# fevzibabaoglu/adaptive-edge-aware-jpeg

Measured on NVIDIA B200. Metric: encode+decode megapixels/sec, higher is better.
Workload: dtype f32

## Files before the change

adaptive-edge-aware-jpeg_b200/csrc/canny.cu:

```cuda
#include "aeaj_internal.cuh"

namespace {

__constant__ float c_bil_color[256];
__constant__ float c_bil_space[13];
__constant__ int c_bil_dy[13];
__constant__ int c_bil_dx[13];

struct ClaheGeom { int th, tw, clip; float lutScale, inv_th, inv_tw; };
__host__ __device__ inline ClaheGeom clahe_geom(int h, int w) {
    int eh = h, ew = w;
    if ((w % 4) != 0 || (h % 4) != 0) { eh = h + (4 - h % 4); ew = w + (4 - w % 4); }
    ClaheGeom g;
    g.th = eh / 4; g.tw = ew / 4;
    int area = g.th * g.tw;
    g.lutScale = 255.0f / (float)area;
    int clip = (int)(0.75 * area / 256);
    g.clip = clip < 1 ? 1 : clip;
    g.inv_th = 1.0f / (float)g.th; g.inv_tw = 1.0f / (float)g.tw;
    return g;
}

constexpr int HIST_ROWS = 32;
__device__ __forceinline__ void hist_add16(unsigned int* wh, uint4 q) {
    const unsigned w[4] = {q.x, q.y, q.z, q.w};
    int prev = w[0] & 0xff, cnt = 0;
#pragma unroll
    for (int k = 0; k < 16; k++) {
        const int v = (w[k >> 2] >> (8 * (k & 3))) & 0xff;
        if (v == prev) cnt++;
        else { atomicAdd(&wh[prev], (unsigned)cnt); prev = v; cnt = 1; }
    }
    atomicAdd(&wh[prev], (unsigned)cnt);
}
__global__ void __launch_bounds__(256) k_clahe_hist(const PlaneDesc* __restrict__ planes) {
    const PlaneDesc& P = planes[blockIdx.z];
    ClaheGeom g = clahe_geom(P.h, P.w);
    const int tile = blockIdx.y, ty = tile >> 2, tx = tile & 3;
    const int r0 = blockIdx.x * HIST_ROWS;
    if (r0 >= g.th) return;
    __shared__ unsigned int wh[8][256];
    for (int i = threadIdx.x; i < 8 * 256; i += 256) (&wh[0][0])[i] = 0;
    __syncthreads();
    const int warp = threadIdx.x >> 5, lane = threadIdx.x & 31;
    const int r1 = min(r0 + HIST_ROWS, g.th);
    const uint8_t* src = P.u8a;
    unsigned int* my = wh[warp];
    const int cx0 = tx * g.tw, cx1 = cx0 + g.tw;
    const int band_hi = (P.ry1 >= P.h) ? 4 * g.th : P.ry1;
    for (int r = r0 + warp; r < r1; r += 8) {
        const int gy = ty * g.th + r;
        if (gy < P.ry0 || gy >= band_hi) continue;
        const int sy = reflect101(gy, P.h);
        const uint8_t* rowp = src + (size_t)sy * P.w;
        const int xa = cx0, xb = min(cx1, P.w);
        if (xa < xb) {
            const int head = min((int)((16 - ((uintptr_t)(rowp + xa) & 15)) & 15), xb - xa);
            const int nvec = (xb - xa - head) >> 4;
            const int tail0 = xa + head + nvec * 16;
            for (int x = xa + lane; x < xa + head; x += 32) atomicAdd(&my[rowp[x]], 1u);
            for (int x = tail0 + lane; x < xb; x += 32) atomicAdd(&my[rowp[x]], 1u);
            const uint4* vp = reinterpret_cast<const uint4*>(rowp + xa + head);
            for (int c = lane; c < nvec; c += 32) hist_add16(my, __ldg(vp + c));
        }
        for (int x = max(cx0, P.w) + lane; x < cx1; x += 32) atomicAdd(&my[rowp[reflect101(x, P.w)]], 1u);
    }
    __syncthreads();
    unsigned s = 0;
#pragma unroll
    for (int k = 0; k < 8; k++) s += wh[k][threadIdx.x];
    if (s) atomicAdd(&P.clahe_hist[tile * 256 + threadIdx.x], s);
}

__device__ __forceinline__ unsigned peer_sum(const unsigned int* mine, const PeerSet& peers) {
    unsigned s = 0;
    for (int r = 0; r < peers.world; r++)
        s += (r == peers.rank) ? *mine : __ldcv(reinterpret_cast<const unsigned int*>(reinterpret_cast<const char*>(mine) + peers.delta[r]));
    return s;
}

__global__ void __launch_bounds__(256) k_clahe_lut(const PlaneDesc* __restrict__ planes, const __grid_constant__ PeerSet peers) {
    const PlaneDesc& P = planes[blockIdx.y];
    ClaheGeom g = clahe_geom(P.h, P.w);
    const int tile = blockIdx.x, i = threadIdx.x;
    __shared__ int red[256];
    int hv = (int)peer_sum(&P.clahe_hist[tile * 256 + i], peers);
    int excess = hv > g.clip ? hv - g.clip : 0;
    hv = hv > g.clip ? g.clip : hv;
    red[i] = excess;
    __syncthreads();
    for (int s = 128; s > 0; s >>= 1) { if (i < s) red[i] += red[i + s]; __syncthreads(); }
    int clipped = red[0];
    __syncthreads();
    int redist = clipped / 256, residual = clipped - redist * 256;
    hv += redist;
    if (residual != 0) {
        int step = 256 / residual; if (step < 1) step = 1;
        if ((i % step) == 0 && (i / step) < residual) hv++;
    }
    red[i] = hv;
    __syncthreads();
    for (int off = 1; off < 256; off <<= 1) {
        int t = (i >= off) ? red[i - off] : 0;
        __syncthreads();
        red[i] += t;
        __syncthreads();
    }
    int v = __float2int_rn(__fmul_rn((float)red[i], g.lutScale));
    P.clahe_lut[tile * 256 + i] = (uint8_t)(v < 0 ? 0 : (v > 255 ? 255 : v));
}

constexpr int PF_TW = 128, PF_TH = 64;
constexpr int PF_CG = PF_TW / 4;
constexpr int PF_CR = 2 * (256 / PF_CG);
constexpr int PF_AS = PF_TW + 8;
constexpr int PF_AG = PF_AS / 4;
#define BIL_TAPS_UP(X) X(0,-2,0,3) X(1,-1,-1,2) X(2,-1,0,1) X(3,-1,1,2) X(4,0,-2,3) X(5,0,-1,1)
#define BIL_TAPS_DN(X) X(7,0,1,1) X(8,0,2,3) X(9,1,-1,2) X(10,1,0,1) X(11,1,1,2) X(12,2,0,3)

__global__ void __launch_bounds__(256, 4) k_prefilter(const PlaneDesc* __restrict__ planes, const __grid_constant__ TileMap tm, int stages, int do_hist) {
    int plane_i, txi, tyi;
    tile_decode(tm, blockIdx.x, plane_i, txi, tyi);
    const PlaneDesc& P = planes[plane_i];
    const int X0 = txi * PF_TW, Y0 = tyi * PF_TH;
    if (Y0 < P.ry0 || Y0 >= P.ry1) return;
    __shared__ __align__(16) uint8_t sA[PF_TH + 6][PF_AS];
    __shared__ __align__(16) uint16_t sG[PF_TH + 4][PF_AS];
    __shared__ __align__(16) uint8_t sLut[16][256];
    __shared__ uint32_t sQuad[4][256];
    __shared__ float sW[4][256];
    __shared__ unsigned int sHist[256];
    __shared__ __align__(16) float sXa[PF_AS];
    __shared__ float sYa[PF_TH + 6];
    __shared__ uint8_t sTx[PF_AS][2], sTy[PF_TH + 6][2];
    __shared__ __align__(16) int sFx[PF_AS];
    __shared__ long long sRow[PF_TH + 6];
    __shared__ __align__(16) int sCo[PF_AS];
    __shared__ int sRo[PF_TH + 6];
    const int tid = threadIdx.x;
    const ClaheGeom g = clahe_geom(P.h, P.w);
    auto tile_of = [](int coord, float inv, float& frac, int& t_lo, int& t_hi) {
        const float tf = __fsub_rn(__fmul_rn((float)coord, inv), 0.5f);
        const int t1 = (int)floorf(tf);
        frac = __fsub_rn(tf, (float)t1);
        t_lo = max(t1, 0); t_hi = min(t1 + 1, 3);
    };
    int two_ok = 1;
    if (tid < PF_AS) {
        const int x = reflect101(X0 + tid - 3, P.w);
        sFx[tid] = x;
        float fr, fr0; int lo, hi, lo0, hi0, loL, hiL;
        tile_of(x, g.inv_tw, fr, lo, hi);
        tile_of(reflect101(X0 - 3, P.w), g.inv_tw, fr0, lo0, hi0);
        tile_of(reflect101(X0 + PF_AS - 4, P.w), g.inv_tw, fr0, loL, hiL);
        sXa[tid] = fr;
        sTx[tid][0] = (uint8_t)lo; sTx[tid][1] = (uint8_t)hi;
        const bool r0 = (lo == lo0 && hi == hi0), r1 = (lo == loL && hi == hiL);
        sCo[tid] = r0 ? 0 : 1024;
        two_ok = r0 || r1;
    } else if (tid >= PF_AS && tid < PF_AS + PF_TH + 6) {
        const int r = tid - PF_AS;
        const int y = reflect101(Y0 + r - 3, P.h);
        sRow[r] = ((y < P.ry0) ? P.peer_up : ((y >= P.ry1) ? P.peer_dn : 0ll)) + (long long)y * P.w;
        float fr, fr0; int lo, hi, lo0, hi0, loL, hiL;
        tile_of(y, g.inv_th, fr, lo, hi);
        tile_of(reflect101(Y0 - 3, P.h), g.inv_th, fr0, lo0, hi0);
        tile_of(reflect101(Y0 + PF_TH + 2, P.h), g.inv_th, fr0, loL, hiL);
        sYa[r] = fr;
        sTy[r][0] = (uint8_t)(lo * 4); sTy[r][1] = (uint8_t)(hi * 4);
        const bool r0 = (lo == lo0 && hi == hi0), r1 = (lo == loL && hi == hiL);
        sRo[r] = r0 ? 0 : 2048;
        two_ok = r0 || r1;
    }
    {
        float cw = c_bil_color[tid];
        sW[0][tid] = cw;
        sW[1][tid] = __fmul_rn(c_bil_space[2], cw);
        sW[2][tid] = __fmul_rn(c_bil_space[1], cw);
        sW[3][tid] = __fmul_rn(c_bil_space[0], cw);
        sHist[tid] = 0;
    }
    const bool uniform = __syncthreads_and(two_ok) != 0;
    const bool clahe = (stages & 1) != 0;
    if (clahe) {
        if (uniform) {
            const uint8_t* l = P.clahe_lut;
            const int rr[2] = {sTy[0][0] * 256, sTy[PF_TH + 5][0] * 256}, rh[2] = {sTy[0][1] * 256, sTy[PF_TH + 5][1] * 256};
            const int cl[2] = {sTx[0][0] * 256, sTx[PF_AS - 1][0] * 256}, ch[2] = {sTx[0][1] * 256, sTx[PF_AS - 1][1] * 256};
            const int nry = (sRo[PF_TH + 5] != 0) ? 2 : 1, ncx = (sCo[PF_AS - 1] != 0) ? 2 : 1;
            for (int ry = 0; ry < nry; ry++)
                for (int cx = 0; cx < ncx; cx++)
                    sQuad[ry * 2 + cx][tid] = (uint32_t)l[rr[ry] + cl[cx] + tid] | ((uint32_t)l[rr[ry] + ch[cx] + tid] << 8) |
                                              ((uint32_t)l[rh[ry] + cl[cx] + tid] << 16) | ((uint32_t)l[rh[ry] + ch[cx] + tid] << 24);
        } else {
            for (int i = tid; i < 16 * 256 / 4; i += 256) reinterpret_cast<uint32_t*>(&sLut[0][0])[i] = reinterpret_cast<const uint32_t*>(P.clahe_lut)[i];
        }
        __syncthreads();
    }
    const uint8_t* src = P.u8a;
    const bool tile_remote = (Y0 - 3 < P.ry0 && P.peer_up != 0) || (Y0 + PF_TH + 3 > P.ry1 && P.peer_dn != 0);
    auto stage_a = [&](auto remote_tag) {
        constexpr bool REMOTE = decltype(remote_tag)::value;
        auto ld8 = [](const uint8_t* p) -> int { return REMOTE ? (int)__ldcv(p) : (int)*p; };
        if (!clahe || uniform) {
            static_assert((PF_TH + 6) % (256 / PF_AG) == 0, "stage A row walk");
            constexpr int RSTEP = 256 / PF_AG;
            if (tid < RSTEP * PF_AG) {
                const int gx = (tid % PF_AG) * 4;
                const int4 fx = *reinterpret_cast<const int4*>(&sFx[gx]);
                const float4 xa4 = *reinterpret_cast<const float4*>(&sXa[gx]);
                const float xav[4] = {xa4.x, xa4.y, xa4.z, xa4.w};
                const float xa1v[4] = {__fsub_rn(1.0f, xa4.x), __fsub_rn(1.0f, xa4.y), __fsub_rn(1.0f, xa4.z), __fsub_rn(1.0f, xa4.w)};
                const int4 co4 = *reinterpret_cast<const int4*>(&sCo[gx]);
                const char* qbase = reinterpret_cast<const char*>(&sQuad[0][0]);
                const int xw = X0 - 4 + gx;
                const bool words = xw >= 0 && xw + 8 <= P.w && (P.w & 3) == 0 && fx.x == xw + 1 && fx.w == xw + 4;
#pragma unroll 2
                for (int ry = tid / PF_AG; ry < PF_TH + 6; ry += RSTEP) {
                    const uint8_t* srow = src + sRow[ry];
                    int v[4];
                    if (words) {
                        const uint32_t* wp = reinterpret_cast<const uint32_t*>(srow + xw);
                        const uint32_t w0 = REMOTE ? __ldcv(wp) : __ldg(wp), w1 = REMOTE ? __ldcv(wp + 1) : __ldg(wp + 1);
                        v[0] = (w0 >> 8) & 0xff; v[1] = (w0 >> 16) & 0xff; v[2] = w0 >> 24; v[3] = w1 & 0xff;
                    } else {
                        v[0] = ld8(srow + fx.x); v[1] = ld8(srow + fx.y); v[2] = ld8(srow + fx.z); v[3] = ld8(srow + fx.w);
                    }
                    uint32_t packed;
                    if (clahe) {
                        int o[4];
                        const float ya = sYa[ry], ya1 = __fsub_rn(1.0f, ya);
                        const int ro = sRo[ry];
                        const int cov[4] = {co4.x + ro, co4.y + ro, co4.z + ro, co4.w + ro};
#pragma unroll
                        for (int k = 0; k < 4; k++) {
                            const uint32_t q = *reinterpret_cast<const uint32_t*>(qbase + cov[k] + v[k] * 4);
                            const float xa = xav[k], xa1 = xa1v[k];
                            const float a = __fmul_rn((float)(q & 0xffu), xa1), b = __fmul_rn((float)((q >> 8) & 0xffu), xa);
                            const float c = __fmul_rn((float)((q >> 16) & 0xffu), xa1), d = __fmul_rn((float)(q >> 24), xa);
                            o[k] = __float2int_rn(__fadd_rn(__fmul_rn(__fadd_rn(a, b), ya1), __fmul_rn(__fadd_rn(c, d), ya)));
                        }
                        packed = __byte_perm(__byte_perm(o[0], o[1], 0x0040), __byte_perm(o[2], o[3], 0x0040), 0x5410);
                    } else {
                        packed = __byte_perm(__byte_perm(v[0], v[1], 0x0040), __byte_perm(v[2], v[3], 0x0040), 0x5410);
                    }
                    *reinterpret_cast<uint32_t*>(&sA[ry][gx]) = packed;
                }
            }
        } else {
            for (int i = tid; i < (PF_TH + 6) * PF_AS; i += 256) {
                const int ry = i / PF_AS, rx = i - ry * PF_AS;
                const int v = ld8(src + sRow[ry] + sFx[rx]);
                const float xa = sXa[rx], xa1 = __fsub_rn(1.0f, xa), ya = sYa[ry], ya1 = __fsub_rn(1.0f, ya);
                const uint8_t* l0 = &sLut[sTy[ry][0]][v];
                const uint8_t* l1 = &sLut[sTy[ry][1]][v];
                const int c0 = sTx[rx][0] * 256, c1 = sTx[rx][1] * 256;
                const float a = __fmul_rn((float)l0[c0], xa1), b = __fmul_rn((float)l0[c1], xa);
                const float c = __fmul_rn((float)l1[c0], xa1), d = __fmul_rn((float)l1[c1], xa);
                const float r = __fadd_rn(__fmul_rn(__fadd_rn(a, b), ya1), __fmul_rn(__fadd_rn(c, d), ya));
                sA[ry][rx] = (uint8_t)min(max(__float2int_rn(r), 0), 255);
            }
        }
    };
    if (tile_remote) stage_a(std::true_type{});
    else stage_a(std::false_type{});
    __syncthreads();
    for (int i = tid; i < (PF_TH + 4) * (PF_CG + 1); i += 256) {
        const int ry = i / (PF_CG + 1), gx = (i - ry * (PF_CG + 1)) * 4;
        if (stages & 2) {
            uint32_t cs[3];
            {
                uint32_t p[3][3];
#pragma unroll
                for (int r = 0; r < 3; r++) {
                    const uint32_t w0 = *reinterpret_cast<const uint32_t*>(&sA[ry + r][gx]), w1 = *reinterpret_cast<const uint32_t*>(&sA[ry + r][gx + 4]);
                    p[r][0] = __byte_perm(w0, 0, 0x4140); p[r][1] = __byte_perm(w0, 0, 0x4342); p[r][2] = __byte_perm(w1, 0, 0x4140);
                }
#pragma unroll
                for (int j = 0; j < 3; j++) cs[j] = p[0][j] + 2 * p[1][j] + p[2][j];
            }
            const uint32_t s1 = __byte_perm(cs[0], cs[1], 0x5432), s3 = __byte_perm(cs[1], cs[2], 0x5432);
            const uint32_t o01 = cs[0] + cs[1] + 0x00080008u + 2 * s1, o23 = cs[1] + cs[2] + 0x00080008u + 2 * s3;
            *reinterpret_cast<uint2*>(&sG[ry][gx]) = make_uint2((o01 >> 2) & 0x03fc03fcu, (o23 >> 2) & 0x03fc03fcu);
        } else {
            int o[4];
#pragma unroll
            for (int k = 0; k < 4; k++) o[k] = sA[ry + 1][gx + 1 + k];
            *reinterpret_cast<uint2*>(&sG[ry][gx]) = make_uint2((uint32_t)(o[0] << 2) | ((uint32_t)(o[1] << 2) << 16), (uint32_t)(o[2] << 2) | ((uint32_t)(o[3] << 2) << 16));
        }
    }
    __syncthreads();
    uint8_t* dst = P.u8b;
    const int tx = (tid % PF_CG) * 4;
#pragma unroll 1
    for (int half = 0; half < PF_TH / PF_CR; half++) {
    const int ty0 = (tid / PF_CG) * 2 + PF_CR * half;
    uint32_t outw[2] = {0, 0};
    {
        int wi[6][8];
#pragma unroll
        for (int r = 0; r < 6; r++) {
            const uint2 a = *reinterpret_cast<const uint2*>(&sG[ty0 + r][tx]);
            const uint2 b = *reinterpret_cast<const uint2*>(&sG[ty0 + r][tx + 4]);
            wi[r][0] = a.x & 0xffffu; wi[r][1] = a.x >> 16; wi[r][2] = a.y & 0xffffu; wi[r][3] = a.y >> 16;
            wi[r][4] = b.x & 0xffffu; wi[r][5] = b.x >> 16; wi[r][6] = b.y & 0xffffu; wi[r][7] = b.y >> 16;
        }
        if (stages & 4) {
            const float w_c = sW[0][0];
            const char* wbase = reinterpret_cast<const char*>(&sW[0][0]);
#define BIL_ONE(idx, dy, dx, cls) { const int v = wi[rr + 2 + (dy)][k + 2 + (dx)]; \
                                    const float wgt = *reinterpret_cast<const float*>(wbase + (cls) * 1024 + __sad(v, v0, 0u)); \
                                    sum = __fmaf_rn((float)v, wgt, sum); wsum = __fadd_rn(wsum, wgt); }
#define BIL_PIXEL { const int v0 = wi[rr + 2][k + 2]; \
                    sum = 0.0f; wsum = 0.0f; \
                    BIL_TAPS_UP(BIL_ONE) \
                    sum = __fmaf_rn((float)v0, w_c, sum); wsum = __fadd_rn(wsum, w_c); \
                    BIL_TAPS_DN(BIL_ONE) }
#pragma unroll
            for (int rr = 0; rr < 2; rr++) {
                constexpr unsigned ins[4] = {0x3214u, 0x3240u, 0x3410u, 0x4210u};
                uint32_t word = 0;
                float worst = 0.0f;
#pragma unroll
                for (int k = 0; k < 4; k++) {
                    float sum, wsum, rw;
                    BIL_PIXEL
                    asm("rcp.approx.ftz.f32 %0, %1;" : "=f"(rw) : "f"(wsum));
                    const float q0 = __fmul_rn(__fmul_rn(sum, rw), 0.25f);
                    const float kf = rintf(q0);
                    word = __byte_perm(word, (uint32_t)(int)kf, ins[k]);
                    worst = fmaxf(worst, fabsf(__fsub_rn(q0, kf)));
                }
                if (worst > 0.499f) {
#pragma unroll
                    for (int k = 0; k < 4; k++) {
                        float sum, wsum;
                        BIL_PIXEL
                        word = __byte_perm(word, (uint32_t)__float2int_rn(__fmul_rn(__fdiv_rn(sum, wsum), 0.25f)), ins[k]);
                    }
                }
                outw[rr] = word;
            }
#undef BIL_PIXEL
#undef BIL_ONE
        } else {
#pragma unroll
            for (int rr = 0; rr < 2; rr++)
#pragma unroll
                for (int k = 0; k < 4; k++) outw[rr] |= (uint32_t)(wi[rr + 2][k + 2] >> 2) << (8 * k);
        }
    }
    const int x = X0 + tx;
#pragma unroll
    for (int rr = 0; rr < 2; rr++) {
        const int y = Y0 + ty0 + rr;
        if (y >= P.h) continue;
        uint8_t* drow = dst + (size_t)y * P.w;
        if (x + 3 < P.w && ((P.w & 3) == 0)) *reinterpret_cast<uint32_t*>(drow + x) = outw[rr];
        else {
#pragma unroll
            for (int k = 0; k < 4; k++) if (x + k < P.w) drow[x + k] = (uint8_t)(outw[rr] >> (8 * k));
        }
        if (do_hist) {
            const uint32_t w = outw[rr], b0 = w & 0xffu;
            if ((x + 3 < P.w) && (w == b0 * 0x01010101u)) {
                atomicAdd(&sHist[b0], 4u);
            } else {
#pragma unroll
                for (int k = 0; k < 4; k++)
                    if (x + k < P.w) atomicAdd(&sHist[(w >> (8 * k)) & 0xffu], 1u);
            }
        }
    }
    }
    if (do_hist) {
        __syncthreads();
        if (sHist[tid]) atomicAdd(&P.hist[tid], sHist[tid]);
    }
}

__global__ void __launch_bounds__(256) k_hist_u8(const uint8_t* __restrict__ src, size_t n, unsigned int* __restrict__ hist) {
    __shared__ unsigned int sh[256];
    sh[threadIdx.x] = 0;
    __syncthreads();
    for (size_t i = (size_t)blockIdx.x * 256 + threadIdx.x; i < n; i += (size_t)gridDim.x * 256) atomicAdd(&sh[src[i]], 1u);
    __syncthreads();
    if (sh[threadIdx.x]) atomicAdd(&hist[threadIdx.x], sh[threadIdx.x]);
}

__device__ void canny_prepare_thresholds(double lo, double hi, int* thr) {
    if (lo > hi) { double t = lo; lo = hi; hi = t; }
    lo = fmin(32767.0, lo); hi = fmin(32767.0, hi);
    if (lo > 0) lo *= lo;
    if (hi > 0) hi *= hi;
    thr[0] = (int)floor(lo); thr[1] = (int)floor(hi);
}
__device__ __forceinline__ int first_bin_above(const unsigned long long* cum8, unsigned long long target, int lane) {
    const unsigned m = __ballot_sync(0xffffffffu, cum8[7] > target);
    const int src = __ffs(m) - 1;
    int bin = 0;
#pragma unroll
    for (int k = 7; k >= 0; k--) if (cum8[k] > target) bin = 8 * lane + k;
    return __shfl_sync(0xffffffffu, bin, src < 0 ? 31 : src);
}
__device__ __forceinline__ double percentile_warp(const unsigned long long* cum8, unsigned long long n, double q, int lane) {
    const double v = (double)(n - 1) * q;
    const double lo = floor(v), gfrac = v - lo;
    const unsigned long long ilo = (unsigned long long)lo, ihi = ilo + 1 < n ? ilo + 1 : n - 1;
    const int a = first_bin_above(cum8, ilo, lane), b = first_bin_above(cum8, ihi, lane);
    const double d = (double)(b - a);
    return gfrac < 0.5 ? (double)a + d * gfrac : (double)b - d * (1.0 - gfrac);
}
__global__ void __launch_bounds__(128) k_thresholds(const PlaneDesc* __restrict__ planes, int nplanes, const __grid_constant__ PeerSet peers) {
    const int p = blockIdx.x * (blockDim.x >> 5) + (threadIdx.x >> 5), lane = threadIdx.x & 31;
    if (p >= nplanes) return;
    const PlaneDesc& P = planes[p];
    unsigned long long cum8[8];
    unsigned long long run = 0;
#pragma unroll
    for (int k = 0; k < 8; k++) { run += peer_sum(&P.hist[8 * lane + k], peers); cum8[k] = run; }
    unsigned long long inc = run;
#pragma unroll
    for (int o = 1; o < 32; o <<= 1) { const unsigned long long t = __shfl_up_sync(0xffffffffu, inc, o); if (lane >= o) inc += t; }
    const unsigned long long off = inc - run;
#pragma unroll
    for (int k = 0; k < 8; k++) cum8[k] += off;
    const unsigned long long n = (unsigned long long)P.h * P.w;
    const double lo = percentile_warp(cum8, n, 10.0 / 100.0, lane), hi = percentile_warp(cum8, n, 30.0 / 100.0, lane);
    if (lane == 0) {
        if (P.thr_d) { P.thr_d[0] = lo; P.thr_d[1] = hi; }
        canny_prepare_thresholds(lo, hi, P.thr);
    }
}
__global__ void k_thresholds_from_double(const double* thr_d, int* thr) { canny_prepare_thresholds(thr_d[0], thr_d[1], thr); }

constexpr int NM_TW = 64, NM_TH = 64;
constexpr int NM_SS = NM_TW + 8;
constexpr int NM_MS = NM_TW + 4;
__device__ __forceinline__ int dp4a_us(uint32_t a, uint32_t b, int c) {
    int d;
    asm("dp4a.u32.s32 %0, %1, %2, %3;" : "=r"(d) : "r"(a), "r"(b), "r"(c));
    return d;
}

__device__ __forceinline__ int selnz(int a, int b, int c) {
    int r;
    asm("{.reg .pred p; setp.ne.s32 p, %3, 0; selp.s32 %0, %1, %2, p;}" : "=r"(r) : "r"(a), "r"(b), "r"(c));
    return r;
}

__global__ void __launch_bounds__(256) k_canny_nms(const PlaneDesc* __restrict__ planes, const __grid_constant__ TileMap tm) {
    int plane_i, txi, tyi;
    tile_decode(tm, blockIdx.x, plane_i, txi, tyi);
    const PlaneDesc& P = planes[plane_i];
    const int X0 = txi * NM_TW, Y0 = tyi * NM_TH;
    if (Y0 < P.ry0 || Y0 >= P.ry1) return;
    __shared__ __align__(16) uint8_t sS[NM_TH + 4][NM_SS];
    __shared__ __align__(16) int sM[NM_TH + 2][NM_MS];
    const int tid = threadIdx.x;
    const uint8_t* src = P.u8b;
    const int ph = P.h, pw = P.w, ry0 = P.ry0, ry1 = P.ry1;
    const long long up = P.peer_up, dn = P.peer_dn;
    const bool tile_remote = (Y0 - 2 < ry0 && up != 0) || (Y0 + NM_TH + 2 > ry1 && dn != 0);
    auto src_row = [&](int y) -> const uint8_t* {
        return src + ((y < ry0) ? up : ((y >= ry1) ? dn : 0ll)) + (size_t)y * pw;
    };
    if (X0 >= 4 && X0 + NM_SS - 4 <= pw && (pw & 3) == 0) {
        if (!tile_remote) {
            for (int i = tid; i < (NM_TH + 4) * (NM_SS / 4); i += 256) {
                const int ry = i / (NM_SS / 4), rw = i - ry * (NM_SS / 4);
                reinterpret_cast<uint32_t*>(&sS[ry][0])[rw] =
                    __ldg(reinterpret_cast<const uint32_t*>(src + (size_t)clampi(Y0 + ry - 2, 0, ph - 1) * pw + X0 - 4) + rw);
            }
        } else {
            for (int i = tid; i < (NM_TH + 4) * (NM_SS / 4); i += 256) {
                const int ry = i / (NM_SS / 4), rw = i - ry * (NM_SS / 4);
                reinterpret_cast<uint32_t*>(&sS[ry][0])[rw] = __ldcv(reinterpret_cast<const uint32_t*>(src_row(clampi(Y0 + ry - 2, 0, ph - 1)) + X0 - 4) + rw);
            }
        }
    } else {
        for (int i = tid; i < (NM_TH + 4) * NM_SS; i += 256) {
            const int ry = i / NM_SS, rx = i - ry * NM_SS;
            const uint8_t* p = src_row(clampi(Y0 + ry - 2, 0, ph - 1)) + clampi(X0 + rx - 4, 0, pw - 1);
            sS[ry][rx] = tile_remote ? __ldcv(p) : *p;
        }
    }
    __syncthreads();
    auto sobel = [&](auto interior_tag) {
        constexpr bool INTERIOR = decltype(interior_tag)::value;
        for (int i = tid; i < (NM_TH + 2) * (NM_MS / 4); i += 256) {
            const int ry = i / (NM_MS / 4), c0 = (i - ry * (NM_MS / 4)) * 4;
            uint32_t wa[3], wb[3];
#pragma unroll
            for (int k = 0; k < 3; k++) {
                wa[k] = *reinterpret_cast<const uint32_t*>(&sS[ry + k][c0]);
                wb[k] = *reinterpret_cast<const uint32_t*>(&sS[ry + k][c0 + 4]);
            }
            int m[4];
            const int y = Y0 - 1 + ry;
            const bool yin = (y >= 0 && y < P.h);
#pragma unroll
            for (int k = 0; k < 4; k++) {
                constexpr unsigned sel[4] = {0x5432u, 0x6543u, 0x7654u, 0x7765u};
                const uint32_t t = __byte_perm(wa[0], wb[0], sel[k]), c = __byte_perm(wa[1], wb[1], sel[k]), b = __byte_perm(wa[2], wb[2], sel[k]);
                const int gx = dp4a_us(b, 0x000100ffu, dp4a_us(c, 0x000200feu, dp4a_us(t, 0x000100ffu, 0)));
                const int gy = dp4a_us(b, 0x00010201u, dp4a_us(t, 0x00fffeffu, 0));
                const int ax = abs(gx), ay = abs(gy) << 15;
                const int tg22x = ax * 13573, tg67x = tg22x + (ax << 16);
                const int nh = ay >= tg22x, dg = nh && !(ay > tg67x), pos = dg && ((gx ^ gy) >= 0);
                int v = ((gx * gx + gy * gy) << 2) + nh + dg + pos;
                if (!INTERIOR) {
                    const int x = X0 - 1 + c0 + k;
                    v = (yin && x >= 0 && x < P.w) ? v : 0;
                }
                m[k] = v;
            }
            *reinterpret_cast<int4*>(&sM[ry][c0]) = make_int4(m[0], m[1], m[2], m[3]);
        }
    };
    if (X0 >= 1 && X0 + NM_MS - 1 <= P.w && Y0 >= 1 && Y0 + NM_TH + 1 <= P.h) sobel(std::true_type{});
    else sobel(std::false_type{});
    __syncthreads();
    const int low4 = min(P.thr[0], 1 << 22) * 4 + 3, high4 = min(P.thr[1], 1 << 22) * 4 + 3;
    const int lane = tid & 31;
    const int gx4 = (tid & 15) * 4;
#pragma unroll 2
    for (int half = 0; half < NM_TH / 16; half++) {
        const int ty = (tid >> 4) + half * 16;
        const int y = Y0 + ty;
        int mg[3][6];
#pragma unroll
        for (int k = 0; k < 3; k++) {
            const int4 a = *reinterpret_cast<const int4*>(&sM[ty + k][gx4]);
            const int2 b = *reinterpret_cast<const int2*>(&sM[ty + k][gx4 + 4]);
            mg[k][0] = a.x; mg[k][1] = a.y; mg[k][2] = a.z; mg[k][3] = a.w; mg[k][4] = b.x; mg[k][5] = b.y;
        }
        unsigned sb = 0, wb = 0;
#pragma unroll
        for (int k = 0; k < 4; k++) {
            const int c = mg[1][k + 1];
            const int d = c & 3;
            const int d1 = d & 1, d2 = d & 2;
            const int n1 = selnz(selnz(mg[0][k], mg[0][k + 2], d1), selnz(mg[0][k + 1], mg[1][k], d1), d2);
            const int n2 = selnz(selnz(mg[2][k + 2], mg[2][k], d1), selnz(mg[2][k + 1], mg[1][k + 2], d1), d2);
            const int c_gt = c & ~3;
            const int c2 = selnz(c_gt - 1, c | 3, d2);
            const int keep = (c > low4) & (c_gt > n1) & (c2 >= n2);
            const int strong = keep & (c > high4);
            sb |= (unsigned)strong << k;
            wb |= (unsigned)(keep ^ strong) << k;
        }
        sb <<= 4 * (lane & 7); wb <<= 4 * (lane & 7);
#pragma unroll
        for (int o = 1; o < 8; o <<= 1) { sb |= __shfl_xor_sync(0xffffffffu, sb, o); wb |= __shfl_xor_sync(0xffffffffu, wb, o); }
        const int word = (X0 + gx4) >> 5;
        if ((lane & 7) == 0 && y < P.h && word < P.wpr) {
            P.strong[(size_t)y * P.wpr + word] = sb;
            P.weak[(size_t)y * P.wpr + word] = wb;
        }
    }
}

constexpr int HY_WW = 8, HY_TR = 32;
constexpr int HY_THREADS = HY_WW * HY_TR;
constexpr int HY_SS = HY_WW + 3;
constexpr int HY_HEAD = 0, HY_TAIL = 32, HY_NEXT = 64, HY_ABORT = 96, HY_AVAIL = 128, HY_CTRL_INTS = 160;
constexpr long long HY_SPIN_LIMIT = 20000000;

struct HystQueue { int* flags; int* ring; int* ctrl; int ring_mask; int ntiles; };

__device__ __forceinline__ unsigned spread3(unsigned L, unsigned Cw, unsigned R) {
    return Cw | (Cw << 1) | (Cw >> 1) | (L >> 31) | (R << 31);
}
__device__ __forceinline__ int ld_gpu(const int* p) {
    int v;
    asm volatile("ld.relaxed.gpu.global.s32 %0, [%1];" : "=r"(v) : "l"(p) : "memory");
    return v;
}

__device__ __forceinline__ void hyst_process_tile(const PlaneDesc* __restrict__ planes, const TileMap& tm, int tile, const HystQueue& q,
                                                  unsigned (*sS)[HY_SS], int* sNbr) {
    const int tid = threadIdx.x, tr = tid & 31, tc = tid >> 5;
    int plane_i, txi, tyi;
    tile_decode(tm, tile, plane_i, txi, tyi);
    const PlaneDesc& P = planes[plane_i];
    const int ntx = aeaj_cdiv(P.wpr, HY_WW);
    const int gy0 = tyi * HY_TR, gw0 = txi * HY_WW;
    __syncthreads();
    if (tid == 0) *sNbr = 0;
    for (int i = tid; i < (HY_TR + 2) * (HY_WW + 2); i += HY_THREADS) {
        const int ry = i / (HY_WW + 2), rw = i - ry * (HY_WW + 2);
        const int gy = gy0 + ry - 1, gw = gw0 + rw - 1;
        unsigned v = 0;
        if (gy >= 0 && gy < P.h && gw >= 0 && gw < P.wpr) v = __ldcg(P.strong + (size_t)gy * P.wpr + gw);
        sS[ry][rw] = v;
    }
    const int gw = gw0 + tc, gy = gy0 + tr;
    const bool inb = (gy < P.h && gw < P.wpr);
    const unsigned wk = inb ? __ldg(P.weak + (size_t)gy * P.wpr + gw) : 0u;
    __syncthreads();
    const unsigned s_init = sS[tr + 1][tc + 1];
    unsigned s = s_init;
    for (;;) {
        const unsigned n = spread3(sS[tr][tc], sS[tr][tc + 1], sS[tr][tc + 2]) |
                           spread3(sS[tr + 1][tc], s, sS[tr + 1][tc + 2]) |
                           spread3(sS[tr + 2][tc], sS[tr + 2][tc + 1], sS[tr + 2][tc + 2]);
        unsigned add = wk & ~s & n;
        unsigned t = s | add;
        while (add) { add = wk & ~t & ((t << 1) | (t >> 1)); t |= add; }
        const int ch = (t != s);
        __syncthreads();
        if (ch) { s = t; sS[tr + 1][tc + 1] = s; }
        if (!__syncthreads_or(ch)) break;
    }
    unsigned nb = 0;
    if (inb && s != s_init) {
        atomicOr(P.strong + (size_t)gy * P.wpr + gw, s);
        const unsigned diff = s ^ s_init;
        const bool L = (tc == 0) && (diff & 1u), R = (tc == HY_WW - 1) && (diff >> 31);
        if (tr == 0) nb |= 2u | (L ? 1u : 0u) | (R ? 4u : 0u);
        if (tr == HY_TR - 1) nb |= 128u | (L ? 64u : 0u) | (R ? 256u : 0u);
        if (L) nb |= 8u;
        if (R) nb |= 32u;
    }
    if (nb) atomicOr(sNbr, (int)nb);
    __syncthreads();
    if (*sNbr == 0) return;
    if (tid == 0) __threadfence();
    __syncthreads();
    if (tid < 9 && tid != 4 && ((*sNbr >> tid) & 1)) {
        const int dy = tid / 3 - 1, dx = tid % 3 - 1;
        const int nx = txi + dx, ny = tyi + dy;
        if (nx >= 0 && nx < ntx && ny >= 0 && ny * HY_TR < P.h) {
            const int nt = tile + dy * ntx + dx;
            if (atomicExch(&q.flags[nt], 1) == 0) {
                const int slot = atomicAdd(&q.ctrl[HY_TAIL], 1) & q.ring_mask;
                long long spins = 0;
                while (atomicCAS(&q.ring[slot], -1, nt) != -1)
                    if (++spins > HY_SPIN_LIMIT) { atomicExch(&q.ctrl[HY_ABORT], 1); break; }
                if (atomicAdd(&q.ctrl[HY_AVAIL], 1) == 0x7fffffff) atomicExch(&q.ctrl[HY_ABORT], 1);
            }
        }
    }
}

__global__ void __launch_bounds__(HY_THREADS) k_hysteresis(const PlaneDesc* __restrict__ planes, const __grid_constant__ TileMap tm, HystQueue q,
                                                           int* __restrict__ status) {
    __shared__ unsigned sS[HY_TR + 2][HY_SS];
    __shared__ int sNbr, sTile;
    const int tid = threadIdx.x;
    for (;;) {
        __syncthreads();
        if (tid == 0) {
            int t = -1;
            if (ld_gpu(&q.ctrl[HY_AVAIL]) > 0) {
                if (atomicSub(&q.ctrl[HY_AVAIL], 1) > 0) {
                    const int slot = atomicAdd(&q.ctrl[HY_HEAD], 1) & q.ring_mask;
                    long long spins = 0;
                    while ((t = ld_gpu(&q.ring[slot])) == -1)
                        if (++spins > HY_SPIN_LIMIT) { atomicExch(&q.ctrl[HY_ABORT], 1); break; }
                    if (t >= 0) atomicExch(&q.ring[slot], -1);
                } else atomicAdd(&q.ctrl[HY_AVAIL], 1);
            }
            if (t < 0 && ld_gpu(&q.ctrl[HY_NEXT]) < q.ntiles) {
                const int f = atomicAdd(&q.ctrl[HY_NEXT], 1);
                if (f < q.ntiles) t = f;
            }
            if (t >= 0 && atomicExch(&q.flags[t], 0) == 0x7fffffff) t = -1;
            sTile = t;
        }
        __syncthreads();
        const int tile = sTile;
        if (tile < 0) break;
        hyst_process_tile(planes, tm, tile, q, sS, &sNbr);
    }
    if (tid == 0 && status) {
        status[0] = ld_gpu(&q.ctrl[HY_TAIL]);
        status[1] = ld_gpu(&q.ctrl[HY_ABORT]) ? 0 : 1;
    }
}

__global__ void __launch_bounds__(256) k_bitmap_to_u8(const PlaneDesc* __restrict__ planes) {
    const PlaneDesc& P = planes[blockIdx.z];
    uint8_t* out = P.tap_edge;
    int x = blockIdx.x * 256 + threadIdx.x, y = blockIdx.y;
    if (!out || y >= P.h || x >= P.w) return;
    out[(size_t)y * P.w + x] = (P.strong[(size_t)y * P.wpr + (x >> 5)] >> (x & 31)) & 1u;
}
__global__ void __launch_bounds__(256) k_u8_to_bitmap(const uint8_t* __restrict__ edge, int h, int w, int wpr, uint32_t* __restrict__ bits) {
    int word = blockIdx.x * 8 + (threadIdx.x >> 5), y = blockIdx.y, lane = threadIdx.x & 31;
    if (word >= wpr) return;
    int x = word * 32 + lane;
    unsigned b = __ballot_sync(0xffffffffu, x < w && edge[(size_t)y * w + x] == 1);
    if (lane == 0) bits[(size_t)y * wpr + word] = b;
}

int max_dim(const PlaneDesc* P, int n, bool width) {
    int m = 0;
    for (int i = 0; i < n; i++) m = std::max(m, width ? P[i].w : P[i].h);
    return m;
}

}

int aeaj_canny_init_constants() {
    float color[256], space[13];
    int dy[13], dx[13];
    double cc = -0.5 / (75.0 * 75.0), sc = -0.5 / (75.0 * 75.0);
    for (int i = 0; i < 256; i++) color[i] = (float)exp((double)(i * i) * cc);
    int k = 0;
    for (int i = -2; i <= 2; i++)
        for (int j = -2; j <= 2; j++) {
            double r = sqrt((double)i * i + (double)j * j);
            if (r > 2) continue;
            space[k] = (float)exp(r * r * sc); dy[k] = i; dx[k] = j; k++;
        }
    AEAJ_CUDA(cudaMemcpyToSymbol(c_bil_color, color, sizeof color));
    AEAJ_CUDA(cudaMemcpyToSymbol(c_bil_space, space, sizeof space));
    AEAJ_CUDA(cudaMemcpyToSymbol(c_bil_dy, dy, sizeof dy));
    AEAJ_CUDA(cudaMemcpyToSymbol(c_bil_dx, dx, sizeof dx));
    return 0;
}

int launch_clahe_hist(const PlaneDesc* planes_dev, const PlaneDesc* P, int nplanes, cudaStream_t st) {
    int maxth = 0;
    for (int i = 0; i < nplanes; i++) maxth = std::max(maxth, clahe_geom(P[i].h, P[i].w).th);
    dim3 grd(aeaj_cdiv(maxth, HIST_ROWS), 16, nplanes);
    k_clahe_hist<<<grd, 256, 0, st>>>(planes_dev);
    AEAJ_LAUNCH_CHECK();
    return 0;
}
int launch_clahe_lut(const PlaneDesc* planes_dev, int nplanes, const PeerSet& peers, cudaStream_t st) {
    k_clahe_lut<<<dim3(16, nplanes), 256, 0, st>>>(planes_dev, peers);
    AEAJ_LAUNCH_CHECK();
    return 0;
}
int launch_prefilter(const PlaneDesc* planes_dev, const PlaneDesc* P, int nplanes, int stages, int do_hist, cudaStream_t st) {
    const TileMap tm = make_tile_map(P, nplanes, PF_TW, PF_TH);
    k_prefilter<<<tile_map_total(tm, nplanes), 256, 0, st>>>(planes_dev, tm, stages, do_hist);
    AEAJ_LAUNCH_CHECK();
    return 0;
}
int launch_hist_u8(const uint8_t* src, size_t n, unsigned int* hist, cudaStream_t st) {
    int blocks = (int)std::min<size_t>((n + 4095) / 4096, 148 * 8);
    k_hist_u8<<<std::max(blocks, 1), 256, 0, st>>>(src, n, hist);
    AEAJ_LAUNCH_CHECK();
    return 0;
}
int launch_thresholds(const PlaneDesc* planes_dev, int nplanes, const PeerSet& peers, cudaStream_t st) {
    k_thresholds<<<aeaj_cdiv(nplanes, 4), 128, 0, st>>>(planes_dev, nplanes, peers);
    AEAJ_LAUNCH_CHECK();
    return 0;
}
int launch_thresholds_from_double(const double* thr_d, int* thr, cudaStream_t st) {
    k_thresholds_from_double<<<1, 1, 0, st>>>(thr_d, thr);
    AEAJ_LAUNCH_CHECK();
    return 0;
}
int launch_canny_nms(const PlaneDesc* planes_dev, const PlaneDesc* P, int nplanes, cudaStream_t st) {
    const TileMap tm = make_tile_map(P, nplanes, NM_TW, NM_TH);
    k_canny_nms<<<tile_map_total(tm, nplanes), 256, 0, st>>>(planes_dev, tm);
    AEAJ_LAUNCH_CHECK();
    return 0;
}

int hysteresis_tiles(PlaneDesc* P, int nplanes, int* ring_cap) {
    const TileMap tm = make_tile_map(P, nplanes, HY_WW * 32, HY_TR);
    const int ns = tile_map_total(tm, nplanes);
    int cap = 64;
    while (cap < 2 * ns) cap *= 2;
    *ring_cap = cap;
    return ns;
}
int hysteresis_ctrl_ints() { return HY_CTRL_INTS; }

int aeaj_canny_init(aeaj_handle* h) {
    int rc = aeaj_canny_init_constants(); if (rc) return rc;
    AEAJ_CUDA(cudaOccupancyMaxActiveBlocksPerMultiprocessor(&h->hyst_blocks_per_sm, k_hysteresis, HY_THREADS, 0));
    if (h->hyst_blocks_per_sm < 1) { aeaj_set_error("hysteresis kernel cannot be resident"); return AEAJ_EINVAL; }
    return 0;
}

int launch_hysteresis(aeaj_handle* h, const PlaneDesc* planes_dev, const PlaneDesc* planes_host, int nplanes, int ntiles, int ring_cap,
                      int* flags, int* ring, int* ctrl, int* status, cudaStream_t st) {
    AEAJ_CUDA(cudaMemsetAsync(flags, 1, sizeof(int) * (size_t)ntiles, st));
    AEAJ_CUDA(cudaMemsetAsync(ring, 0xff, sizeof(int) * (size_t)ring_cap, st));
    AEAJ_CUDA(cudaMemsetAsync(ctrl, 0, sizeof(int) * HY_CTRL_INTS, st));
    HystQueue q;
    q.flags = flags; q.ring = ring; q.ctrl = ctrl; q.ring_mask = ring_cap - 1; q.ntiles = ntiles;
    const TileMap tm = make_tile_map(planes_host, nplanes, HY_WW * 32, HY_TR);
    const int grid = std::max(1, std::min(ntiles, h->hyst_blocks_per_sm * h->sm_count));
    k_hysteresis<<<grid, HY_THREADS, 0, st>>>(planes_dev, tm, q, status);
    AEAJ_LAUNCH_CHECK();
    return 0;
}

int launch_bitmap_to_u8(const PlaneDesc* planes_dev, const PlaneDesc* P, int nplanes, cudaStream_t st) {
    dim3 grd(aeaj_cdiv(max_dim(P, nplanes, true), 256), max_dim(P, nplanes, false), nplanes);
    k_bitmap_to_u8<<<grd, 256, 0, st>>>(planes_dev);
    AEAJ_LAUNCH_CHECK();
    return 0;
}
int launch_u8_to_bitmap(const uint8_t* edge, int h, int w, uint32_t* bits, cudaStream_t st) {
    int wpr = aeaj_cdiv(w, 32);
    k_u8_to_bitmap<<<dim3(aeaj_cdiv(wpr, 8), h), 256, 0, st>>>(edge, h, w, wpr, bits);
    AEAJ_LAUNCH_CHECK();
    return 0;
}
```

Baseline: 28580.

## Vectorize bilateral filter with paired f32x2 math and magic-number int/float conversion

Replaces integer-to-float conversions (I2F) and float rounding (F2I/rint) with byte_perm magic-number tricks using the 2^23 exponent bias. The bilateral filter now processes two output rows at once with packed float2 FMA/add instructions (__ffma2_rn, __fadd2_rn). Unpacked pixel values are no longer held in a 6x8 int register array. In the rare fallback path the values are reloaded from shared memory through volatile loads. The aim is to cut ALU instruction count and register pressure in the prefilter kernel. The price is more complex code and some risk of exact-rounding differences.

Measured after the change: 28860, median of 6. About the same (+1.0%).

```diff
diff --git a/adaptive-edge-aware-jpeg_b200/csrc/canny.cu b/adaptive-edge-aware-jpeg_b200/csrc/canny.cu
--- a/adaptive-edge-aware-jpeg_b200/csrc/canny.cu
+++ b/adaptive-edge-aware-jpeg_b200/csrc/canny.cu
@@ -117,6 +117,14 @@
 constexpr int PF_AG = PF_AS / 4;
 #define BIL_TAPS_UP(X) X(0,-2,0,3) X(1,-1,-1,2) X(2,-1,0,1) X(3,-1,1,2) X(4,0,-2,3) X(5,0,-1,1)
 #define BIL_TAPS_DN(X) X(7,0,1,1) X(8,0,2,3) X(9,1,-1,2) X(10,1,0,1) X(11,1,1,2) X(12,2,0,3)
+
+constexpr float F_2P23 = 8388608.0f, F_ROUND = 12582912.0f;
+constexpr uint32_t BITS_2P23 = 0x4B000000u;
+__device__ __forceinline__ uint32_t magic_bits(uint32_t w, uint32_t sel) { return __byte_perm(w, BITS_2P23, sel); }
+__device__ __forceinline__ float2 u8_to_f2(uint32_t w, uint32_t sel_x, uint32_t sel_y) {
+    return __fadd2_rn(make_float2(__uint_as_float(magic_bits(w, sel_x)), __uint_as_float(magic_bits(w, sel_y))), make_float2(-F_2P23, -F_2P23));
+}
+__device__ __forceinline__ uint32_t round_bits(float x) { return __float_as_uint(__fadd_rn(x, F_ROUND)); }
 
 __global__ void __launch_bounds__(256, 4) k_prefilter(const PlaneDesc* __restrict__ planes, const __grid_constant__ TileMap tm, int stages, int do_hist) {
     int plane_i, txi, tyi;
@@ -236,9 +244,10 @@
                         for (int k = 0; k < 4; k++) {
                             const uint32_t q = *reinterpret_cast<const uint32_t*>(qbase + cov[k] + v[k] * 4);
                             const float xa = xav[k], xa1 = xa1v[k];
-                            const float a = __fmul_rn((float)(q & 0xffu), xa1), b = __fmul_rn((float)((q >> 8) & 0xffu), xa);
-                            const float c = __fmul_rn((float)((q >> 16) & 0xffu), xa1), d = __fmul_rn((float)(q >> 24), xa);
-                            o[k] = __float2int_rn(__fadd_rn(__fmul_rn(__fadd_rn(a, b), ya1), __fmul_rn(__fadd_rn(c, d), ya)));
+                            const float2 l02 = u8_to_f2(q, 0x7440u, 0x7442u), l13 = u8_to_f2(q, 0x7441u, 0x7443u);
+                            const float a = __fmul_rn(l02.x, xa1), b = __fmul_rn(l13.x, xa);
+                            const float c = __fmul_rn(l02.y, xa1), d = __fmul_rn(l13.y, xa);
+                            o[k] = (int)round_bits(__fadd_rn(__fmul_rn(__fadd_rn(a, b), ya1), __fmul_rn(__fadd_rn(c, d), ya)));
                         }
                         packed = __byte_perm(__byte_perm(o[0], o[1], 0x0040), __byte_perm(o[2], o[3], 0x0040), 0x5410);
                     } else {
@@ -297,57 +306,74 @@
     const int ty0 = (tid / PF_CG) * 2 + PF_CR * half;
     uint32_t outw[2] = {0, 0};
     {
-        int wi[6][8];
+        uint32_t wr[6][4];
 #pragma unroll
         for (int r = 0; r < 6; r++) {
             const uint2 a = *reinterpret_cast<const uint2*>(&sG[ty0 + r][tx]);
             const uint2 b = *reinterpret_cast<const uint2*>(&sG[ty0 + r][tx + 4]);
-            wi[r][0] = a.x & 0xffffu; wi[r][1] = a.x >> 16; wi[r][2] = a.y & 0xffffu; wi[r][3] = a.y >> 16;
-            wi[r][4] = b.x & 0xffffu; wi[r][5] = b.x >> 16; wi[r][6] = b.y & 0xffffu; wi[r][7] = b.y >> 16;
-        }
+            wr[r][0] = a.x; wr[r][1] = a.y; wr[r][2] = b.x; wr[r][3] = b.y;
+        }
+        auto eb = [&](int r, int c) { return magic_bits(wr[r][c >> 1], (c & 1) ? 0x7432u : 0x7410u); };
         if (stages & 4) {
             const float w_c = sW[0][0];
             const char* wbase = reinterpret_cast<const char*>(&sW[0][0]);
-#define BIL_ONE(idx, dy, dx, cls) { const int v = wi[rr + 2 + (dy)][k + 2 + (dx)]; \
-                                    const float wgt = *reinterpret_cast<const float*>(wbase + (cls) * 1024 + __sad(v, v0, 0u)); \
-                                    sum = __fmaf_rn((float)v, wgt, sum); wsum = __fadd_rn(wsum, wgt); }
-#define BIL_PIXEL { const int v0 = wi[rr + 2][k + 2]; \
-                    sum = 0.0f; wsum = 0.0f; \
-                    BIL_TAPS_UP(BIL_ONE) \
-                    sum = __fmaf_rn((float)v0, w_c, sum); wsum = __fadd_rn(wsum, w_c); \
-                    BIL_TAPS_DN(BIL_ONE) }
+            auto wgt = [&](int cls, uint32_t e, uint32_t e0) { return *reinterpret_cast<const float*>(wbase + cls * 1024 + __sad(e, e0, 0u)); };
+            constexpr unsigned ins[4] = {0x3214u, 0x3240u, 0x3410u, 0x4210u};
+            float worst[2] = {0.0f, 0.0f};
+#pragma unroll
+            for (int k = 0; k < 4; k++) {
+                const uint32_t c0 = eb(2, k + 2), c1 = eb(3, k + 2);
+                auto vpair = [&](int r, int c) {
+                    return __fadd2_rn(make_float2(__uint_as_float(eb(r, c)), __uint_as_float(eb(r + 1, c))), make_float2(-F_2P23, -F_2P23));
+                };
+                float2 sum = make_float2(0.0f, 0.0f), wsum = sum;
+#define BIL_TWO(idx, dy, dx, cls) { const float2 w = make_float2(wgt(cls, eb(2 + (dy), k + 2 + (dx)), c0), wgt(cls, eb(3 + (dy), k + 2 + (dx)), c1)); \
+                                    sum = __ffma2_rn(vpair(2 + (dy), k + 2 + (dx)), w, sum); wsum = __fadd2_rn(wsum, w); }
+                BIL_TAPS_UP(BIL_TWO)
+                sum = __ffma2_rn(vpair(2, k + 2), make_float2(w_c, w_c), sum); wsum = __fadd2_rn(wsum, make_float2(w_c, w_c));
+                BIL_TAPS_DN(BIL_TWO)
+#undef BIL_TWO
+                float2 rw;
+                asm("rcp.approx.ftz.f32 %0, %1;" : "=f"(rw.x) : "f"(wsum.x));
+                asm("rcp.approx.ftz.f32 %0, %1;" : "=f"(rw.y) : "f"(wsum.y));
+                const float2 q0 = __fmul2_rn(__fmul2_rn(sum, rw), make_float2(0.25f, 0.25f));
+                const float2 t = __fadd2_rn(q0, make_float2(F_ROUND, F_ROUND));
+                const float2 kf = __fadd2_rn(t, make_float2(-F_ROUND, -F_ROUND));
+                const float2 d = __ffma2_rn(kf, make_float2(-1.0f, -1.0f), q0);
+                outw[0] = __byte_perm(outw[0], __float_as_uint(t.x), ins[k]);
+                outw[1] = __byte_perm(outw[1], __float_as_uint(t.y), ins[k]);
+                worst[0] = fmaxf(worst[0], fabsf(d.x));
+                worst[1] = fmaxf(worst[1], fabsf(d.y));
+            }
 #pragma unroll
             for (int rr = 0; rr < 2; rr++) {
-                constexpr unsigned ins[4] = {0x3214u, 0x3240u, 0x3410u, 0x4210u};
-                uint32_t word = 0;
-                float worst = 0.0f;
-#pragma unroll
-                for (int k = 0; k < 4; k++) {
-                    float sum, wsum, rw;
-                    BIL_PIXEL
-                    asm("rcp.approx.ftz.f32 %0, %1;" : "=f"(rw) : "f"(wsum));
-                    const float q0 = __fmul_rn(__fmul_rn(sum, rw), 0.25f);
-                    const float kf = rintf(q0);
-                    word = __byte_perm(word, (uint32_t)(int)kf, ins[k]);
-                    worst = fmaxf(worst, fabsf(__fsub_rn(q0, kf)));
+                if (worst[rr] > 0.499f) {
+                    uint32_t wx[6][4];
+#pragma unroll
+                    for (int r = 0; r < 6; r++)
+#pragma unroll
+                        for (int j = 0; j < 4; j++) wx[r][j] = reinterpret_cast<const volatile uint32_t*>(&sG[ty0 + r][tx])[j];
+                    auto xb = [&](int r, int c) { return magic_bits(wx[r][c >> 1], (c & 1) ? 0x7432u : 0x7410u); };
+                    auto ef = [&](int r, int c) { return __fsub_rn(__uint_as_float(xb(r, c)), F_2P23); };
+#define BIL_ONE(idx, dy, dx, cls) { const float w = wgt(cls, xb(rr + 2 + (dy), k + 2 + (dx)), c0); \
+                                    sum = __fmaf_rn(ef(rr + 2 + (dy), k + 2 + (dx)), w, sum); wsum = __fadd_rn(wsum, w); }
+#pragma unroll
+                    for (int k = 0; k < 4; k++) {
+                        const uint32_t c0 = xb(rr + 2, k + 2);
+                        float sum = 0.0f, wsum = 0.0f;
+                        BIL_TAPS_UP(BIL_ONE)
+                        sum = __fmaf_rn(ef(rr + 2, k + 2), w_c, sum); wsum = __fadd_rn(wsum, w_c);
+                        BIL_TAPS_DN(BIL_ONE)
+                        outw[rr] = __byte_perm(outw[rr], (uint32_t)__float2int_rn(__fmul_rn(__fdiv_rn(sum, wsum), 0.25f)), ins[k]);
+                    }
+#undef BIL_ONE
                 }
-                if (worst > 0.499f) {
-#pragma unroll
-                    for (int k = 0; k < 4; k++) {
-                        float sum, wsum;
-                        BIL_PIXEL
-                        word = __byte_perm(word, (uint32_t)__float2int_rn(__fmul_rn(__fdiv_rn(sum, wsum), 0.25f)), ins[k]);
-                    }
-                }
-                outw[rr] = word;
-            }
-#undef BIL_PIXEL
-#undef BIL_ONE
+            }
         } else {
 #pragma unroll
             for (int rr = 0; rr < 2; rr++)
 #pragma unroll
-                for (int k = 0; k < 4; k++) outw[rr] |= (uint32_t)(wi[rr + 2][k + 2] >> 2) << (8 * k);
+                for (int k = 0; k < 4; k++) outw[rr] |= ((eb(rr + 2, k + 2) & 0xffffu) >> 2) << (8 * k);
         }
     }
     const int x = X0 + tx;
```
